# raahii/dcvgan

Hardware: AMD Instinct MI355X
Metric: videos/sec per G+D step, 16x64x64 RGB+depth (higher is better)
Workload: dtype f32

## Files before the change

### dcvgan_amd/csrc/conv_mfma.hip

```cpp
#include "dcv_common.h"

#include <algorithm>
#include <cstdlib>
#include <map>
#include <mutex>
#include <string>
#include <type_traits>
#include <vector>

namespace dcv {

thread_local char g_err[512] = {0};
std::atomic<uint64_t> g_launches{0};
thread_local char g_last_kernel[160] = {0};
#define DCV_NOTE_KERNEL(...) snprintf(g_last_kernel, sizeof(g_last_kernel), __VA_ARGS__)

typedef float f32x16 __attribute__((ext_vector_type(16)));
typedef __bf16 bf16x8 __attribute__((ext_vector_type(8)));

std::atomic<int> g_precision{0};
struct BnView {
    const float* bx; const float* gamma; const float* beta; const float* mean; const float* invstd;
    int64_t bx_sn;
    int32_t bx_sc, bx_sh, cbn, act;
    float slope;
};

__device__ __forceinline__ bf16x8 pack_bf16x8(const float (&t)[8]) {
// ... 1661 lines not shown
                if (accumulate) { v[0] += dst[0]; v[1] += dst[1]; }
                dst[0] = apply_act(v[0], act, slope);
                dst[1] = apply_act(v[1], act, slope);
            }
}

template <int T>
static bool launch_thin_struct(const GatherArgs& a, int OC, int RC, int rc_per_split, dim3 grid, hipStream_t s) {
    switch (OC) {
        case 1: hipLaunchKernelGGL((thin_struct_kernel<T, 1>), grid, dim3(256), 0, s, a, RC, rc_per_split); return true;
        case 2: hipLaunchKernelGGL((thin_struct_kernel<T, 2>), grid, dim3(256), 0, s, a, RC, rc_per_split); return true;
        case 3: hipLaunchKernelGGL((thin_struct_kernel<T, 3>), grid, dim3(256), 0, s, a, RC, rc_per_split); return true;
        case 4: hipLaunchKernelGGL((thin_struct_kernel<T, 4>), grid, dim3(256), 0, s, a, RC, rc_per_split); return true;
    }
    return false;
}

struct PackArgs {
    const KEntry* ktab[4];
    float* wp[4];
    int32_t K16[4];
    int32_t fmt[4];
};
__global__ void pack_weights_kernel(const float* __restrict__ w, const PackArgs pa, int OC, int OCp, int64_t ws_o) {
    const int c = blockIdx.y;
    const int64_t i = (int64_t)blockIdx.x * blockDim.x + threadIdx.x;
    if (i >= (int64_t)pa.K16[c] * OCp) return;
    const int k = (int)(i / OCp), oc = (int)(i % OCp);
    const KEntry e = pa.ktab[c][k];
    float v = 0.f;
    if (oc < OC && !(e.tapsel >> 31)) v = w[(int64_t)oc * ws_o + e.w_off];
    if (pa.fmt[c] == 2) {
        if (X6_PHASE(k >> 4)) v = -v;
        __bf16* o = reinterpret_cast<__bf16*>(pa.wp[c]);
        const __bf16 hi = (__bf16)v;
        const float r = v - (float)hi;
        const __bf16 mid = (__bf16)r;
        const __bf16 lo = (__bf16)(r - (float)mid);
        const int64_t base = (((int64_t)(k >> 4) * 6 + ((k >> 3) & 1)) * OCp + oc) * 8 + (k & 7);
        o[base] = hi; o[base + (int64_t)2 * OCp * 8] = mid; o[base + (int64_t)4 * OCp * 8] = lo;
    } else if (pa.fmt[c]) reinterpret_cast<__bf16*>(pa.wp[c])[((int64_t)(k >> 3) * OCp + oc) * 8 + (k & 7)] = (__bf16)v;
    else pa.wp[c][i] = v;
}

struct WgradArgs {
    const float* dptr;
    const float* gptr;
    float* slab;
    const KEntry* jtab;
    int32_t M, DC, J, DCp, Jp, chunk, pad0, pad1;
    FastDiv div_sp, div_hw, div_w;
    DimTaps td, th, tw;
    int64_t d_sn, g_sn;
    int32_t d_sc4, d_sd, d_sh, d_sw;
    int32_t g_sd, g_sh, g_sw, pad2;
    int32_t g_sc4, g_sd4, log2nd, pad3;
    int32_t hw_off4[16];
    uint32_t hw_sel[16];
};

template <int TD, int TJ, int WD, int WJ, bool REG16>
__global__ __launch_bounds__(256, (TD * TJ >= 4 ? (REG16 ? 3 : 2) : 3)) void wgrad_gemm_kernel(const WgradArgs a) {
    constexpr int BD = 32 * TD * WD;
    constexpr int BJ = 32 * TJ * WJ;
    constexpr int DPT = BD / 8, JPT = BJ / 8;
// ... 1035 lines not shown
            if (lane == 0 && c0 + cc < a.C)
                out[(int64_t)(c0 + cc) * (ND * 16) + (e >> 2) * 16 + ((1 - ph) + 2 * ((e >> 1) & 1)) * 4 + (1 - pw) + 2 * (e & 1)] = v;
        }
}
#undef DCV_HEAD_LANES

struct DevTable {
    KEntry* dev = nullptr;
    int32_t* koff = nullptr;
    uint32_t* ksel = nullptr;
    int rows = 0;
};

static std::mutex g_plan_mu;
static std::map<std::string, DevTable> g_tables;

struct Toggles {
    bool no_lds_dma, no_dstep, no_patch, no_row64, no_widen, no_widen_mfma, no_thinj_wgrad, no_wgrad_dma, no_wgrad_dma64, no_quad, no_thin_wgrad;
    int half_m;
    bool no_ragged, no_wgrad_d16, no_head_kernels, no_stem3d_wgrad, wgrad_x6;
    int stem3d_stages;
#ifdef DCV_DEBUG_TIMING
    bool debug_nostore;
#endif
    Toggles() {
        auto on = [](const char* n) { return getenv(n) != nullptr; };
        no_lds_dma = on("DCV_NO_LDS_DMA"); no_dstep = on("DCV_NO_DSTEP"); no_patch = on("DCV_NO_PATCH"); no_row64 = on("DCV_NO_ROW64");
        no_widen = on("DCV_NO_WIDEN"); no_widen_mfma = on("DCV_NO_WIDEN_MFMA"); no_thinj_wgrad = on("DCV_NO_THINJ_WGRAD"); no_wgrad_dma = on("DCV_NO_WGRAD_DMA"); no_wgrad_dma64 = on("DCV_NO_WGRAD_DMA64"); no_quad = on("DCV_NO_QUAD"); no_thin_wgrad = on("DCV_NO_THIN_WGRAD");
        half_m = getenv("DCV_HALF_M") ? atoi(getenv("DCV_HALF_M")) : -1;
        no_ragged = on("DCV_NO_RAGGED");
        no_wgrad_d16 = on("DCV_NO_WGRAD_D16");
        no_head_kernels = on("DCV_NO_HEAD_KERNELS"); no_stem3d_wgrad = on("DCV_NO_STEM3D_WGRAD"); wgrad_x6 = on("DCV_WGRAD_X6");
        stem3d_stages = getenv("DCV_STEM3D_STAGES") ? atoi(getenv("DCV_STEM3D_STAGES")) : 0;
#ifdef DCV_DEBUG_TIMING
        debug_nostore = on("DCV_DEBUG_NOSTORE");
#endif
    }
};
static const Toggles& toggles() {
    static const Toggles t;
    return t;
}

struct HeadBnRequest {
    int mode;
    const float* bx; dcv_dims5 bxd; float* bdx; dcv_dims5 bdxd;
    const float* gamma; const float* beta; const float* mean; const float* invstd;
    const float* cst; float* partial; size_t partial_bytes;
    int cbn; float slope;
};

struct CallOpts {
    int precision = 0;
    int wgrad_acc = 0;
    const BnView* bnview = nullptr;
    const HeadBnRequest* headbn = nullptr;
};
static int call_opts(const dcv_conv_geom* g, CallOpts* o, const char* tag) {
// ... 622 lines not shown
        GatherArgsPack one;
        for (int i = 0; i < 4; ++i) one.c[i] = a;
        hipLaunchKernelGGL(splitk_reduce_kernel, dim3((unsigned)((tot + 255) / 256), 1), dim3(256), 0, stream, one, KS2);
        break;
    }
    }
    DCV_LAUNCH_CHECK();
    return DCV_OK;
}

static int run_gather(const GatherOp& op, const GatherPlan& P, const CallOpts& o, const dcv_wpack* pack, void* ws, hipStream_t stream) {
    const TileCfg& tc = P.tc;
    const bool own_pack = pack && pack->buf;
    char* const wp_base = static_cast<char*>(own_pack ? pack->buf : ws);
    const bool pk_ready = own_pack && pack->ready;
    if (P.stat_memset) DCV_HIP_CHECK(hipMemsetAsync(op.stat, 0, P.stat_need, stream));
    GatherArgsPack pend;
    PackArgs packs;
    memset(&packs, 0, sizeof(packs));
    int npack = 0, packmax = 0, npend = 0, KSpend = 1;
    dim3 pend_grid(0, 1, 1);
    auto flush_pk = [&]() {
        if (npack == 0) return (int)DCV_OK;
        const int rc = flush_packs(op.w, packs, npack, packmax, op.OC, P.OCp, op.ws_o, stream);
        npack = packmax = 0;
        return rc;
    };
    auto flush_pend = [&]() {
        int rc = flush_pk();
        if (rc == DCV_OK && npend > 0) rc = flush_pending(pend, npend, pend_grid, tc, KSpend, op.OC, o.precision, stream);
        npend = 0;
        return rc;
    };
    for (const ClassPlan& cp : P.cls) {
        DevTable tab;
        int rc = gather_table(op, cp, &tab);
        if (rc != DCV_OK) return rc;
        GatherArgs a = cp.a;
        float* const wp = reinterpret_cast<float*>(wp_base + cp.wp_off);
        a.x = op.x; a.y = op.y; a.wp = wp; a.koff = tab.koff; a.ksel = tab.ksel; a.gate = op.gate;
        a.slab = cp.KS2 > 1 ? reinterpret_cast<float*>(static_cast<char*>(ws) + cp.slab_off) : nullptr;
        a.stat = cp.stat ? op.stat : nullptr;
        if (!pk_ready) {
            packs.ktab[npack] = tab.dev; packs.wp[npack] = wp; packs.K16[npack] = a.KIT * 16; packs.fmt[npack] = cp.fmt;
            packmax = std::max(packmax, a.KIT * 16);
            if (++npack == 4 && (rc = flush_pk()) != DCV_OK) return rc;
// ... 760 lines not shown
    HeadBnRequest hb{1, bn_x, *bn_xd, bn_dx, *bn_dxd, gamma, beta, save_mean, save_invstd, cst, static_cast<float*>(ws2), pbytes, cbn, act == DCV_ACT_LEAKY ? slope : 1.f};
    o.headbn = &hb;
    ConvCall c; ConvPlan P;
    c.which = 1; c.g = g; c.xd = dxd; c.yd = dyd; c.src = dy; c.w = w; c.dst = dx; c.pack = pack;
    if ((rc = plan_conv(c, o, &P)) != DCV_OK) return rc;
    const bool fuse = P.path == ConvPath::Gather && P.gp.cls.size() == 1 && P.gp.cls[0].kind == GK::HeadBn;
    if ((rc = run_conv(c, P, o, ws, ws_bytes, stream)) != DCV_OK || !fuse) return rc;
    const double count = (double)bn_xd->n * bn_xd->d * bn_xd->h * bn_xd->w;
    hipLaunchKernelGGL(head_bn_finalize_kernel, dim3(cbn), dim3(256), 0, static_cast<hipStream_t>(stream), hb.partial, (int)P.gp.cls[0].grid.x, cbn, count, gamma, save_invstd, dgamma, dbeta, cst);
    DCV_LAUNCH_CHECK();
    hb.mode = 2;
    dcv_wpack pk2;
    if (pack && pack->buf) { pk2 = *pack; pk2.ready = 1; c.pack = &pk2; }
    if ((rc = run_conv(c, P, o, ws, ws_bytes, stream)) != DCV_OK) return rc;
    *fused = 1;
    return DCV_OK;
}

size_t dcv_conv_packed_bytes(const dcv_conv_geom* g, const dcv_dims5* x, const dcv_dims5* y, int which) {
    ConvPlan P;
    return (which == 0 || which == 1) && plan_sizes(g, x, y, which, false, &P) == DCV_OK ? P.gp.pack_need : 0;
}

int dcv_conv_forward(const dcv_conv_geom* g, const float* x, const dcv_dims5* xd, const float* w, float* y, const dcv_dims5* yd,
                     int act, float slope, const dcv_wpack* pack, void* ws, size_t ws_bytes, void* stream) {
    ConvCall c;
    c.g = g; c.xd = xd; c.yd = yd; c.src = x; c.w = w; c.dst = y; c.act = act; c.slope = slope; c.pack = pack;
    return conv_call(c, ws, ws_bytes, stream);
}

size_t dcv_conv_stats_bytes(const dcv_conv_geom* g, const dcv_dims5* x, const dcv_dims5* y) {
    ConvPlan P;
    return plan_sizes(g, x, y, 0, true, &P) == DCV_OK && P.op.stats ? P.gp.stat_need : 0;
}

int dcv_conv_forward_stats(const dcv_conv_geom* g, const float* x, const dcv_dims5* xd, const float* w, float* y, const dcv_dims5* yd,
                           float* stat, size_t stat_bytes, int* nparts, int* pitch, const dcv_wpack* pack, void* ws, size_t ws_bytes, void* stream) {
    if (!stat || !nparts || !pitch) return fail(DCV_EINVAL, "conv_forward_stats: null pointer");
    CallOpts o; ConvCall c; ConvPlan P;
    int rc = call_opts(g, &o, "conv");
    if (rc != DCV_OK) return rc;
    c.g = g; c.xd = xd; c.yd = yd; c.src = x; c.w = w; c.dst = y; c.pack = pack;
    c.stats = true; c.stat = stat; c.stat_bytes = stat_bytes;
    if ((rc = plan_conv(c, o, &P)) != DCV_OK) return rc;
    *pitch = P.gp.OCp;
    return run_conv(c, P, o, ws, ws_bytes, stream, nparts);
// ... 84 lines not shown
```

### dcvgan_amd/native.py

```python
from __future__ import annotations

import ctypes as C
import os
import threading
from typing import Optional, Sequence

import torch

_HERE = os.path.dirname(os.path.abspath(__file__))
LIB_PATH = os.environ.get("DCV_LIB_PATH") or os.path.join(_HERE, "libdcvgan_hip.so")

ACT_NONE, ACT_LEAKY, ACT_TANH = 0, 1, 2
DCV_OK, DCV_EINVAL, DCV_EWORKSPACE, DCV_EHIP, DCV_EUNSUPPORTED = 0, -1, -2, -3, -4


class NativeError(RuntimeError):
    pass


class Dims5(C.Structure):
    _fields_ = [("n", C.c_int32), ("c", C.c_int32), ("d", C.c_int32), ("h", C.c_int32), ("w", C.c_int32),
                ("sn", C.c_int64), ("sc", C.c_int64), ("sd", C.c_int64), ("sh", C.c_int64), ("sw", C.c_int64)]


class WPack(C.Structure):
    _fields_ = [("buf", C.c_void_p), ("bytes", C.c_size_t), ("ready", C.c_int32),
                ("precision", C.c_int32)]


class ConvGeom(C.Structure):
    _fields_ = [("kd", C.c_int32), ("kh", C.c_int32), ("kw", C.c_int32),
                ("sd", C.c_int32), ("sh", C.c_int32), ("sw", C.c_int32),
                ("pd", C.c_int32), ("ph", C.c_int32), ("pw", C.c_int32),
                ("transposed", C.c_int32), ("cin", C.c_int32), ("cout", C.c_int32),
                ("mfma", C.c_int32)]

    def key(self):
        return tuple(getattr(self, f) for f, _ in self._fields_)


class AugLimits(C.Structure):
    _fields_ = [("mx", C.c_int32), ("my", C.c_int32), ("size", C.c_int32), ("mask", C.c_int32), ("contrast", C.c_float), ("brightness", C.c_float)]


class AugWarpLimits(C.Structure):
    _fields_ = [("scale_max", C.c_float), ("aniso_max", C.c_float), ("rot_tan_half", C.c_float), ("frac", C.c_float), ("sat", C.c_float), ("mask", C.c_int32)]


_P = C.c_void_p
_D = C.POINTER(Dims5)
_G = C.POINTER(ConvGeom)
_SIGS = {
    "dcv_last_error": (C.c_char_p, []),
    "dcv_version": (C.c_int, []),
    "dcv_abi_struct_sizes": (None, [C.POINTER(C.c_size_t)]),
    "dcv_conv_effective_precision": (C.c_int, [_G]),
    "dcv_launch_count": (C.c_uint64, []),
    "dcv_debug_kernel_info": (C.c_int, [C.c_char_p, C.c_size_t]),
    "dcv_debug_last_kernel": (C.c_char_p, []),
    "dcv_set_precision": (C.c_int, [C.c_int]),
    "dcv_get_precision": (C.c_int, []),
    "dcv_conv_workspace_bytes": (C.c_size_t, [_G, _D, _D, C.c_int]),
    "dcv_conv_packed_bytes": (C.c_size_t, [_G, _D, _D, C.c_int]),
    "dcv_conv_forward": (C.c_int, [_G, _P, _D, _P, _P, _D, C.c_int, C.c_float, _P, _P, C.c_size_t, _P]),
    "dcv_conv_stats_bytes": (C.c_size_t, [_G, _D, _D]),
    "dcv_conv_forward_stats": (C.c_int, [_G, _P, _D, _P, _P, _D, _P, C.c_size_t, C.POINTER(C.c_int), C.POINTER(C.c_int), _P, _P, C.c_size_t, _P]),
    "dcv_conv_backward_data": (C.c_int, [_G, _P, _D, _P, _P, _D, C.c_int, _P, _P, C.c_size_t, _P]),
    "dcv_conv_backward_data_gated": (C.c_int, [_G, _P, _D, _P, _P, _D, C.c_int, _P, _D, C.c_int, C.c_float, _P, _P, C.c_size_t, _P]),
    "dcv_bn_forward_stats_only": (C.c_int, [_P, _D, _P, _P, _P, _P, _P, C.c_float, C.c_float, _P, C.c_int, C.c_int, _P]),
    "dcv_bn_apply": (C.c_int, [_P, _D, _P, _D, _P, _P, _P, _P, _P, C.c_int, C.c_float, _P]),
    "dcv_conv_forward_bn": (C.c_int, [_G, _P, _D, _P, _P, _D, C.c_int, C.c_float, _P, _P, C.c_size_t, C.c_int, _P, _D, _P, _P, _P, _P, C.c_int, C.c_float, _P]),
    "dcv_conv_backward_weight_bn": (C.c_int, [_G, _P, _D, _P, _D, _P, C.c_int, _P, C.c_size_t, C.c_int, _P, _D, _P, _P, _P, _P, C.c_int, C.c_float, _P]),
    "dcv_conv_backward_data_bn_workspace_bytes": (C.c_size_t, [_D, C.c_int]),
    "dcv_conv_backward_data_bn": (C.c_int, [_G, _P, _D, _P, _P, _D, _P, _P, C.c_size_t, C.c_int, _P, _D, _P, _P, _P, _P, C.c_int, C.c_float, _P, _D, _P, _P,
                                            _P, C.c_size_t, C.POINTER(C.c_int), _P]),
    "dcv_conv_backward_weight": (C.c_int, [_G, _P, _D, _P, _D, _P, _P, C.c_size_t, _P]),
    "dcv_conv_backward_weight_acc": (C.c_int, [_G, _P, _D, _P, _D, _P, C.c_int, _P, C.c_size_t, _P]),
    "dcv_bn_workspace_bytes": (C.c_size_t, [C.c_int]),
    "dcv_bn_act_forward": (C.c_int, [_P, _D, _P, _D, _P, _P, _P, _P, _P, _P, _P, _P, C.c_int, C.c_float, C.c_float, C.c_int, C.c_float, _P, C.c_size_t, _P]),
    "dcv_bn_act_forward_stats": (C.c_int, [_P, _D, _P, _D, _P, _P, _P, _P, _P, _P, _P, _P, C.c_float, C.c_float, C.c_int, C.c_float, _P, C.c_int, C.c_int, _P, C.c_size_t, _P]),
    "dcv_bn_act_backward": (C.c_int, [_P, _D, _P, _D, _P, _D, _P, _P, _P, _P, _P, C.c_int, C.c_int, C.c_float, _P, _P, _P, C.c_size_t, _P]),
    "dcv_act_forward": (C.c_int, [_P, _D, _P, _D, C.c_int, C.c_float, _P]),
    "dcv_act_backward": (C.c_int, [_P, _D, _P, _D, _P, _D, C.c_int, C.c_float, _P]),
    "dcv_axpby": (C.c_int, [_P, _D, C.c_float, _P, _D, C.c_float, _P, _D, _P]),
    "dcv_noise_add": (C.c_int, [_P, _D, _P, _D, C.c_float, C.c_uint64, C.c_uint64, _P]),
    "dcv_normal_fill": (C.c_int, [_P, C.c_int64, C.c_uint64, C.c_uint64, _P]),
# ... 242 lines not shown
```

### dcvgan_amd/ops.py

```python
from __future__ import annotations

import collections
import ctypes as C
import os
from typing import Optional, Tuple

import torch
from torch.autograd import Function

from . import native as N
from .native import ACT_LEAKY, ACT_NONE, ACT_TANH, ConvGeom, check, dims5, lib, ptr, stream_ptr

__all__ = ["invalidate_packed_weights", "conv", "bn_act", "sync_bn_act", "act", "noise_add", "cat_channels", "temporal_diff", "gan_loss", "gru_sequence",
           "normal", "dropout2d_mask", "conv_geom", "ACT_NONE", "ACT_LEAKY", "ACT_TANH"]


def _dense(t: torch.Tensor) -> torch.Tensor:
    if any(s == 0 and n > 1 for s, n in zip(t.stride(), t.shape)):
        return t.contiguous()
    return t


_POISON = bool(int(os.environ.get("DCV_DEBUG_POISON", "0")))
_USE_PACK_CACHE = os.environ.get("DCV_NO_PACK_CACHE") is None
_WGRAD_SIDE = os.environ.get("DCV_NO_WGRAD_SIDE") is None
_HEAD_BN_DEFER = os.environ.get("DCV_NO_HEAD_BN_DEFER") is None
_SKIP_ACCUMULATE = True
_GATED_DGRAD = True
_OWN_ACCUMULATION = True
_HEAD_BN_FUSION = True


def _empty(shape, device) -> torch.Tensor:
    if _POISON:
        return torch.full(tuple(shape), float("nan"), dtype=torch.float32, device=device)
    return torch.empty(tuple(shape), dtype=torch.float32, device=device)
# ... 38 lines not shown
class _Opaque:
    __slots__ = ("v",)

    def __init__(self, v):
        self.v = v


def _dest(out, shape, device):
    if out is None:
        return _empty(shape, device)
    t = out.t
    if tuple(t.shape) != tuple(shape):
        raise N.NativeError(f"out= has shape {tuple(t.shape)}, expected {tuple(shape)}")
    N._require(t, "out= destination")
    return t.detach()


class _PackCache:
    __slots__ = ("entries",)

    def __init__(self):
        self.entries = {}

    def get(self, w, which, g, xd_t, yd_t, xd, yd):
        prec = lib().dcv_conv_effective_precision(C.byref(g))
        key = (which, g.key(), prec, tuple(xd_t.shape), tuple(xd_t.stride()), tuple(yd_t.shape), tuple(yd_t.stride()))
        e = self.entries.get(key)
        stamp = (w._version, w.data_ptr(), prec)
        if _POISON:
            wd = w.detach().double()
            stamp = stamp + (float(wd.sum()), float(wd.abs().sum()))
        if e is None:
            nbytes = lib().dcv_conv_packed_bytes(C.byref(g), C.byref(xd), C.byref(yd), which)
            if nbytes == 0:
                return None
            e = self.entries[key] = [None, torch.empty(nbytes, dtype=torch.uint8, device=w.device), None, None]
        ready = e[0] == stamp
        if w.is_cuda:
            cur = torch.cuda.current_stream(w.device)
            if e[2] is not None and e[3] != cur.cuda_stream:
                cur.wait_event(e[2])
        e[0] = None
        pk = N.WPack(e[1].data_ptr(), e[1].numel(), int(ready), prec)
        pk._entry, pk._stamp, pk._packs = e, stamp, not ready
        return pk

    @staticmethod
    def commit(pk):
        if pk is not None:
            e = pk._entry
            e[0] = pk._stamp
            if pk._packs and e[1].is_cuda:
                cur = torch.cuda.current_stream(e[1].device)
                if e[2] is None:
                    e[2] = torch.cuda.Event()
                e[2].record(cur)
                e[3] = cur.cuda_stream


def _pack_of(w):
    if not _USE_PACK_CACHE:
        return None
    pc = getattr(w, "_dcv_pack", None)
    if pc is None:
        pc = w._dcv_pack = _PackCache()
    return pc


def invalidate_packed_weights(obj) -> None:
    ts = obj.parameters() if isinstance(obj, torch.nn.Module) else [obj]
    for t in ts:
        if getattr(t, "_dcv_pack", None) is not None:
            t._dcv_pack = None


def _task_id() -> int:
    return torch._C._current_graph_task_id()


def _engine_accumulates(p) -> bool:
    tid = _task_id()
    if tid < 0:
        return True
    c = getattr(p, "_dcv_engine", None)
    if c is not None and c[0] == tid:
        return c[1]
    with torch.enable_grad():
        node = p.view_as(p).grad_fn.next_functions[0][0]
    try:
        ok = bool(torch._C._will_engine_execute_node(node))
    except RuntimeError:
        ok = False
    p._dcv_engine = (tid, ok)
    return ok


# ... 809 lines not shown
```

### dcvgan_amd/optim.py

```python
from __future__ import annotations

import ctypes as C
from typing import Iterable, List, Optional

import torch

from .native import NativeError, PointerTable, _require, c_array, check, lib, ptr, stream_ptr


class GradGuard:

    FIELDS = ("loss_scale", "growth_tracker", "grad_norm", "clip_coef", "factor", "skipped", "skipped_total", "nonfinite")

    def __init__(self, max_norm: Optional[float] = None, skip_nonfinite: bool = True, loss_scale: float = 1.0, dynamic: bool = False,
                 growth_factor: float = 2.0, backoff_factor: float = 0.5, growth_interval: int = 2000):
        import math
        if max_norm is not None and not (float(max_norm) > 0.0 and math.isfinite(float(max_norm))):
            raise ValueError(f"GradGuard: max_norm must be a positive finite number or None, got {max_norm!r}")
        if not (float(loss_scale) > 0.0 and math.isfinite(float(loss_scale))):
            raise ValueError(f"GradGuard: loss_scale must be positive and finite, got {loss_scale!r}")
        if not float(growth_factor) > 1.0:
            raise ValueError(f"GradGuard: growth_factor must be > 1, got {growth_factor!r}")
        if not 0.0 < float(backoff_factor) < 1.0:
            raise ValueError(f"GradGuard: backoff_factor must be in (0, 1), got {backoff_factor!r}")
# ... 59 lines not shown
            w.inner.grad_scale = 1.0 / w.world
        scales = {o.grad_scale for o in self.optimizers}
        if len(scales) != 1:
            raise NativeError(f"GradGuard: the registered optimisers disagree on grad_scale ({sorted(scales)})")
        gs, ns, keep = [], [], []
        for o in self.optimizers:
            for p in o.params:
                g = p.grad
                if g is None or g.numel() == 0:
                    continue
                _require(g, "GradGuard gradient")
                g = g.contiguous()
                gs.append(g.data_ptr()); ns.append(g.numel()); keep.append(g)
        tab = self._tables = PointerTable.cached(self._tables, (tuple(gs), tuple(ns)),
                                                 lambda: dict(n=len(gs), g=c_array(gs), numel=c_array(ns, C.c_int64)))
        L = lib()
        need = L.dcv_grad_guard_workspace_bytes(sum(ns), tab.n)
        if self._ws is None or self._ws.numel() < need:
            self._ws = torch.empty(need, dtype=torch.uint8, device=state.device)
        check(L.dcv_grad_guard_measure(tab.n, tab.g, tab.numel, scales.pop(), self.max_norm if self.max_norm is not None else 0.0, int(self.skip_nonfinite), int(self.dynamic),
                                       self.growth_factor, self.backoff_factor, self.growth_interval, ptr(state), ptr(self._ws), self._ws.numel(), stream_ptr()),
              "dcv_grad_guard_measure")
        self.measurements += 1


class Adam:
    def __init__(self, params: Iterable[torch.nn.Parameter], lr: float = 1e-3, betas=(0.9, 0.999), eps: float = 1e-8, weight_decay: float = 0.0,
                 guard: Optional[GradGuard] = None):
        self.params: List[torch.nn.Parameter] = [p for p in params]
        if not self.params:
            raise ValueError("optimizer got an empty parameter list")
        self.lr, self.betas, self.eps, self.weight_decay = float(lr), (float(betas[0]), float(betas[1])), float(eps), float(weight_decay)
        self.state = {}
        self.grad_scale = 1.0
        self.guard = guard
        if guard is not None:
            guard._register(self)

    def zero_grad(self, set_to_none: bool = True):
        for p in self.params:
            if set_to_none:
                p.grad = None
            elif p.grad is not None:
                p.grad.zero_()

    def state_dict(self):
# ... 51 lines not shown
        groups, touched, fresh = {}, [], None
        for p in self.params:
            g = p.grad
            if g is None:
                continue
            _require(p.data, "Adam parameter")
            if not p.data.is_contiguous():
                raise NativeError("Adam: parameters must be contiguous")
            g = g.contiguous()
            s = self.state.get(p)
            if s is None:
                if fresh is None:
                    fresh = torch.zeros(16, dtype=torch.int32, device=p.device)
                s = self.state[p] = {"step": fresh[0], "step_block": fresh, "exp_avg": torch.zeros_like(p.data), "exp_avg_sq": torch.zeros_like(p.data)}
            touched.append(p)
            grp = groups.setdefault(s["step_block"].data_ptr(), ([], [], [], [], [], []))
            grp[0].append(p.data.data_ptr()); grp[1].append(g.data_ptr()); grp[2].append(s["exp_avg"].data_ptr()); grp[3].append(s["exp_avg_sq"].data_ptr())
            grp[4].append(p.numel()); grp[5].append(g)
        for block, (ps, gs, ms, vs, ns, _) in groups.items():
            check(L.dcv_adam_step_multi_guarded(len(ps), c_array(ps), c_array(gs), c_array(ms), c_array(vs), c_array(ns, C.c_int64), self.lr, self.betas[0], self.betas[1],
                                                self.eps, self.weight_decay, C.c_void_p(block), ptr(guard.state), st), "dcv_adam_step_multi_guarded")
        if touched:
            torch.autograd.graph.increment_version(touched)

    @torch.no_grad()
    def step(self):
        if self.guard is not None:
            return self._step_guarded()
        L = lib()
        st = stream_ptr()
        ps, gs, ms, vs, ns, keep = [], [], [], [], [], []
        touched = []
        step = None
        for p in self.params:
            g = p.grad
            if g is None:
                continue
            _require(p.data, "Adam parameter")
            if not p.data.is_contiguous():
                raise NativeError("Adam: parameters must be contiguous")
            g = g.contiguous()
            s = self.state.get(p)
            if s is None:
                s = self.state[p] = {"step": 0, "exp_avg": torch.zeros_like(p.data), "exp_avg_sq": torch.zeros_like(p.data)}
            s["step"] += 1
            touched.append(p)
            if step is None:
                step = s["step"]
            if s["step"] != step:
                check(L.dcv_adam_step(ptr(p.data), ptr(g), ptr(s["exp_avg"]), ptr(s["exp_avg_sq"]), p.numel(), self.lr, self.betas[0], self.betas[1],
                                      self.eps, self.weight_decay, s["step"], self.grad_scale, st), "dcv_adam_step")
                continue
            ps.append(p.data.data_ptr()); gs.append(g.data_ptr()); ms.append(s["exp_avg"].data_ptr()); vs.append(s["exp_avg_sq"].data_ptr())
            ns.append(p.numel()); keep.append(g)
        if ps:
            check(L.dcv_adam_step_multi(len(ps), c_array(ps), c_array(gs), c_array(ms), c_array(vs), c_array(ns, C.c_int64), self.lr, self.betas[0], self.betas[1],
                                        self.eps, self.weight_decay, step, self.grad_scale, st), "dcv_adam_step_multi")
        if touched:
            torch.autograd.graph.increment_version(touched)


class ModelEma:

    def __init__(self, models, names=("ggen", "cgen"), decay: float = 0.999, warmup: bool = True, guard: Optional[GradGuard] = None):
        if not 0.0 <= float(decay) < 1.0:
            raise ValueError(f"ModelEma: decay must be in [0, 1), got {decay!r}")
        self.names = tuple(names)
        if not self.names:
            raise ValueError("ModelEma: no model names")
        self.decay, self.warmup, self.guard = float(decay), bool(warmup), guard
        from .rng import PhiloxRng
        self.live = {n: models[n] for n in self.names}
        self.rng = PhiloxRng()
        self.twins = {n: self._twin(m, self.rng) for n, m in self.live.items()}
        self._pairs = {}
        for n, m in self.live.items():
            tp, tb = dict(self.twins[n].named_parameters()), dict(self.twins[n].named_buffers())
            self._pairs[n] = [(tp[k], p) for k, p in m.named_parameters()] + [(tb[k], b) for k, b in m.named_buffers()]
        self._n_params = {n: sum(1 for _ in m.parameters()) for n, m in self.live.items()}
        self._tables = {}
        dev = next(self.live[self.names[0]].parameters()).device
        self._blocks = {n: torch.zeros(16, dtype=torch.int32).to(dev) for n in self.names}
# ... 504 lines not shown
                _require(t.data, f"SpectralNorm tensor of convolution {i}")
                if not t.is_contiguous():
                    raise NativeError("SpectralNorm: tensors must be contiguous")
            w, w_sn, u, v, sg = row
            if w_sn.shape != w.shape or u.numel() != w.shape[0] or v.numel() != w[0].numel() or sg.numel() != 1:
                raise NativeError(f"SpectralNorm: the buffers of convolution {i} do not fit its weight {tuple(w.shape)}")
        n = len(ts)
        w, w_sn, u, v, sigma = (c_array(col) for col in zip(*ts))
        rows, cols = c_array([row[0].shape[0] for row in ts], C.c_int32), c_array([row[0][0].numel() for row in ts], C.c_int32)
        need = lib().dcv_spectral_workspace_bytes(n, rows, cols)
        if need == 0:
            raise NativeError("dcv_spectral_workspace_bytes: " + lib().dcv_last_error().decode(errors="replace"))
        if self._ws is None or self._ws.numel() < need:
            self._ws = torch.empty(need, dtype=torch.uint8, device=ts[0][0].device)
        return dict(n=n, w=w, w_sn=w_sn, u=u, v=v, sigma=sigma, rows=rows, cols=cols, touched=[row[1] for row in ts])

    @torch.no_grad()
    def update(self, n_iter: int = 1, _guarded: bool = True):
        t = self._table()
        state = ptr(self.guard._need_state()) if (self.guard is not None and _guarded) else None
        check(lib().dcv_spectral_update_multi(t.n, t.w, t.w_sn, t.u, t.v, t.sigma, t.rows, t.cols, int(n_iter), self.eps, state, ptr(self._ws), self._ws.numel(),
                                              stream_ptr()), "dcv_spectral_update_multi")
        torch.autograd.graph.increment_version(t.touched)
        for c in self.convs:
            c.__dict__["_dcv_spectral"].version = c.weight._version

    def refresh(self):
        self.update(n_iter=0, _guarded=False)

    @torch.no_grad()
    def project(self):
        for w in list(self._dp) + (list(self.guard._dp) if self.guard is not None else []):
            w.reduce_gradients()
        t = self._table()
        idx, gs = [], []
        for i, c in enumerate(self.convs):
            g = c.weight.grad
            if g is None:
                continue
            _require(g, "SpectralNorm gradient")
            if not g.is_contiguous() or g.shape != c.weight.shape:
                raise NativeError("SpectralNorm: gradients must be contiguous and of the weight's shape")
            idx.append(i); gs.append(g.data_ptr())
        if not idx:
            return
        pick = lambda arr, ty=C.c_void_p: c_array([arr[i] for i in idx], ty)
# ... 27 lines not shown
```

### dcvgan_amd/trainer.py

```python
from __future__ import annotations

import collections
import os
from typing import Dict, Optional

import torch

from . import discriminator as D
from . import generator as G
from . import loss as Lm
from . import ops, optim, util
from .configs import StepConfig

MODEL_NAMES = ("ggen", "cgen", "idis", "vdis", "gdis")


def build_models(cfg: StepConfig, device=None, sync_bn: bool = False) -> Dict[str, torch.nn.Module]:
    w = cfg.width
    ggen = G.GeometricVideoGenerator(cfg.dim_z_content, cfg.dim_z_motion, cfg.channel, cfg.geometric_info, w["ggen"], cfg.video_length)
    cgen = G.ColorVideoGenerator(ggen.channel, cfg.dim_z_color, cfg.geometric_info, w["cgen"], cfg.video_length)
    idis = D.ImageDiscriminator(ggen.channel, cgen.channel, cfg.use_noise["idis"], cfg.noise_sigma["idis"], w["idis"])
    vdis = D.VideoDiscriminator(ggen.channel, cgen.channel, cfg.use_noise["vdis"], cfg.noise_sigma["vdis"], w["vdis"])
    gdis = D.GradientDiscriminator(ggen.channel, cgen.channel, cfg.use_noise["gdis"], cfg.noise_sigma["gdis"], w["gdis"])
    models = dict(ggen=ggen, cgen=cgen, idis=idis, vdis=vdis, gdis=gdis)
# ... 202 lines not shown
            xg_fake, xc_fake = self._colour(cgen, xg_fake, t_rand)
        self._mark("D: generators forward (beside D on the real batch)")
        y_fake = self._fakes_through(dis, idis, xg_fake, xc_fake, t_rand)
        self._adopt(y_real)
        if self.augment is not None:
            for y in y_real:
                self.augment.observe(y)
        self._mark("D: discriminators forward on the fakes")
        if self.lecam is not None:
            loss_idis, loss_vdis, loss_gdis = self.lecam.compute_dis_losses(self.loss, y_real, y_fake)
        else:
            loss_idis = self.loss.compute_dis_loss(y_real[0], y_fake[0])
            loss_vdis = self.loss.compute_dis_loss(y_real[1], y_fake[1])
            loss_gdis = self.loss.compute_dis_loss(y_real[2], y_fake[2])
        loss_dis = ops.sum_scalars(loss_idis, loss_vdis, loss_gdis) if loss_idis.is_cuda else loss_idis + loss_vdis + loss_gdis
        d_steps = self.iteration % c.num_gen_update == 0
        if d_steps:
            loss_dis.backward(guard_dis.root(loss_dis) if guard_dis is not None else self._root(loss_dis))
            self._mark("D: backward (D lanes, then the generators' dead backward)")
            if self.spectral is not None:
                self.spectral.project()
            if guard_dis is not None:
                guard_dis.measure()
            o["idis"].step(); o["vdis"].step(); o["gdis"].step()
            if self.spectral is not None:
                self.spectral.update()
            self._mark("D: Adam")
        else:
            loss_dis.detach_()
        if self.sync_losses:
            out = {"loss_idis": loss_idis.cpu().item(), "loss_vdis": loss_vdis.cpu().item(), "loss_gdis": loss_gdis.cpu().item()}
        else:
            out = {"loss_idis": loss_idis.detach(), "loss_vdis": loss_vdis.detach(), "loss_gdis": loss_gdis.detach()}
        if self.lecam is not None:
            reg = self.lecam.reg.cpu().tolist() if self.sync_losses else self.lecam.reg
            out["lecam_idis"], out["lecam_vdis"], out["lecam_gdis"] = reg[0], reg[1], reg[2]
        if guard_dis is not None:
            self._guard_report(out, guard_dis, "dis")
        if self.augment is not None:
            self.augment.end_of_iteration(self.iteration)
        if self.monitor is not None:
            seen = {f"{n}_real": y.detach() for n, y in zip(("idis", "vdis", "gdis"), y_real)}
            seen.update({f"{n}_fake_d": y.detach() for n, y in zip(("idis", "vdis", "gdis"), y_fake)})
        del y_real, y_fake, xg_fake, xc_fake, loss_dis
        ggen.train(); cgen.train()
        ggen.zero_grad(); cgen.zero_grad()
        xg_fake = ggen.sample_videos(c.batchsize)
        xg_fake, xc_fake = self._colour(cgen, xg_fake, t_rand)
        self._mark("G: generators forward")
        y_fake = self._fakes_through(dis, idis, xg_fake, xc_fake, t_rand)
        loss_gen = self.loss.compute_gen_loss(*y_fake)
        self._mark("G: discriminators forward on the fakes")
        g_steps = self.iteration % c.num_dis_update == 0
        if g_steps:
            loss_gen.backward(guard_gen.root(loss_gen) if guard_gen is not None else self._root(loss_gen))
            self._mark("G: backward (D lanes, then the generators)")
            if guard_gen is not None:
                guard_gen.measure()
            o["ggen"].step(); o["cgen"].step(); o["ggen"].step()
            if self.ema is not None:
                self.ema.update()
            self._mark("G: Adam")
        else:
            loss_gen.detach_()
        out["loss_gen"] = loss_gen.cpu().item() if self.sync_losses else loss_gen.detach()
        if guard_gen is not None:
            self._guard_report(out, guard_gen, "gen")
        if self.monitor is not None:
            seen.update({f"{n}_fake_g": y.detach() for n, y in zip(("idis", "vdis", "gdis"), y_fake)})
            gated = ([] if d_steps else ["grad_norm_dis", "skipped_dis"]) + ([] if g_steps else ["grad_norm_gen", "skipped_gen"])
            self.monitor.observe({k: v for k, v in out.items() if k not in gated}, seen)
            if self.iteration % self.monitor.interval == 0:
                self.monitor.roll(self.iteration)
            del seen
        if xc_real.is_cuda:
            e = torch.cuda.Event()
            e.record(torch.cuda.current_stream())
            self._inflight.append(e)
        return out
```

### include/dcvgan_hip.h

```cpp
#ifndef DCVGAN_HIP_H
#define DCVGAN_HIP_H

#include <stddef.h>
#include <stdint.h>

#ifdef __cplusplus
extern "C" {
#endif

#define DCV_OK 0
#define DCV_EINVAL (-1)
#define DCV_EWORKSPACE (-2)
#define DCV_EHIP (-3)
#define DCV_EUNSUPPORTED (-4)

#define DCV_ACT_NONE 0
#define DCV_ACT_LEAKY 1
#define DCV_ACT_TANH 2

typedef struct dcv_dims5 {
    int32_t n, c, d, h, w;
    int64_t sn, sc, sd, sh, sw;
} dcv_dims5;

// ... 4 lines not shown
    int32_t transposed;
    int32_t cin, cout;
    int32_t mfma;
} dcv_conv_geom;

const char* dcv_last_error(void);
int dcv_version(void);
void dcv_abi_struct_sizes(size_t out[3]);
uint64_t dcv_launch_count(void);
int dcv_set_precision(int mode);
int dcv_get_precision(void);
int dcv_conv_effective_precision(const dcv_conv_geom* g);
const char* dcv_debug_last_kernel(void);
int dcv_debug_kernel_info(char* buf, size_t n);

size_t dcv_conv_workspace_bytes(const dcv_conv_geom* g, const dcv_dims5* x, const dcv_dims5* y, int which );
typedef struct dcv_wpack {
    float* buf;
    size_t bytes;
    int32_t ready;
    int32_t precision;
} dcv_wpack;
size_t dcv_conv_packed_bytes(const dcv_conv_geom* g, const dcv_dims5* x, const dcv_dims5* y, int which );
int dcv_conv_forward(const dcv_conv_geom* g, const float* x, const dcv_dims5* xd, const float* w,
                     float* y, const dcv_dims5* yd, int act, float slope, const dcv_wpack* pack,
                     void* ws, size_t ws_bytes, void* stream);
size_t dcv_conv_stats_bytes(const dcv_conv_geom* g, const dcv_dims5* x, const dcv_dims5* y);
int dcv_conv_forward_stats(const dcv_conv_geom* g, const float* x, const dcv_dims5* xd, const float* w, float* y, const dcv_dims5* yd,
                           float* stat, size_t stat_bytes, int* nparts, int* pitch, const dcv_wpack* pack, void* ws, size_t ws_bytes, void* stream);
int dcv_conv_backward_data(const dcv_conv_geom* g, const float* dy, const dcv_dims5* dyd, const float* w,
                           float* dx, const dcv_dims5* dxd, int accumulate, const dcv_wpack* pack,
                           void* ws, size_t ws_bytes, void* stream);
int dcv_conv_backward_data_gated(const dcv_conv_geom* g, const float* dy, const dcv_dims5* dyd, const float* w,
                                 float* dx, const dcv_dims5* dxd, int accumulate,
                                 const float* x, const dcv_dims5* xd, int act, float slope, const dcv_wpack* pack,
                                 void* ws, size_t ws_bytes, void* stream);
int dcv_bn_forward_stats_only(const float* x, const dcv_dims5* xd, float* running_mean, float* running_var, int64_t* num_batches_tracked, float* save_mean, float* save_invstd,
                              float momentum, float eps, const float* stat, int nparts, int pitch, void* stream);
int dcv_bn_apply(const float* x, const dcv_dims5* xd, float* y, const dcv_dims5* yd, const float* gamma, const float* beta, const float* save_mean, const float* save_invstd,
                 const float* mask, int act, float slope, void* stream);
int dcv_conv_forward_bn(const dcv_conv_geom* g, const float* x, const dcv_dims5* xd, const float* w, float* y, const dcv_dims5* yd, int act, float slope,
                        const dcv_wpack* pack, void* ws, size_t ws_bytes, int cbn, const float* bn_x, const dcv_dims5* bn_xd, const float* gamma, const float* beta,
                        const float* save_mean, const float* save_invstd, int bn_act, float bn_slope, void* stream);
int dcv_conv_backward_weight_bn(const dcv_conv_geom* g, const float* x, const dcv_dims5* xd, const float* dy, const dcv_dims5* dyd, float* dw, int accumulate,
                                void* ws, size_t ws_bytes, int cbn, const float* bn_x, const dcv_dims5* bn_xd, const float* gamma, const float* beta,
                                const float* save_mean, const float* save_invstd, int bn_act, float bn_slope, void* stream);
// ... 306 lines not shown
```

Measured before the change: 661.2.

## Batch weight repacking into one multi-job kernel launched after optimizer steps

Adds dcv_conv_pack_many, which repacks every cached conv weight touched by the Adam and spectral steps in a single launch. A cached device job table is binary-searched per block. The optimizers call refresh_packed and the trainer groups them with refresh_group, so the per-conv pack launches that used to run lazily inside the next forward pass are skipped. This trades many small launches and their host overhead for one grouped launch, plus extra bookkeeping (stamps and refresh counts) in the pack cache.

```diff
diff --git a/dcvgan_amd/csrc/conv_mfma.hip b/dcvgan_amd/csrc/conv_mfma.hip
--- a/dcvgan_amd/csrc/conv_mfma.hip
+++ b/dcvgan_amd/csrc/conv_mfma.hip
@@ -4,6 +4,7 @@
 #include <cstdlib>
 #include <map>
 #include <mutex>
+#include <set>
 #include <string>
 #include <type_traits>
 #include <vector>
@@ -1711,25 +1712,49 @@
     int32_t K16[4];
     int32_t fmt[4];
 };
-__global__ void pack_weights_kernel(const float* __restrict__ w, const PackArgs pa, int OC, int OCp, int64_t ws_o) {
-    const int c = blockIdx.y;
-    const int64_t i = (int64_t)blockIdx.x * blockDim.x + threadIdx.x;
-    if (i >= (int64_t)pa.K16[c] * OCp) return;
+__device__ __forceinline__ void pack_weights_element(const float* __restrict__ w, const KEntry* __restrict__ ktab, float* __restrict__ wp, int K16, int fmt,
+                                                     int OC, int OCp, int64_t ws_o, int64_t i) {
+    if (i >= (int64_t)K16 * OCp) return;
     const int k = (int)(i / OCp), oc = (int)(i % OCp);
-    const KEntry e = pa.ktab[c][k];
+    const KEntry e = ktab[k];
     float v = 0.f;
     if (oc < OC && !(e.tapsel >> 31)) v = w[(int64_t)oc * ws_o + e.w_off];
-    if (pa.fmt[c] == 2) {
+    if (fmt == 2) {
         if (X6_PHASE(k >> 4)) v = -v;
-        __bf16* o = reinterpret_cast<__bf16*>(pa.wp[c]);
+        __bf16* o = reinterpret_cast<__bf16*>(wp);
         const __bf16 hi = (__bf16)v;
         const float r = v - (float)hi;
         const __bf16 mid = (__bf16)r;
         const __bf16 lo = (__bf16)(r - (float)mid);
         const int64_t base = (((int64_t)(k >> 4) * 6 + ((k >> 3) & 1)) * OCp + oc) * 8 + (k & 7);
         o[base] = hi; o[base + (int64_t)2 * OCp * 8] = mid; o[base + (int64_t)4 * OCp * 8] = lo;
-    } else if (pa.fmt[c]) reinterpret_cast<__bf16*>(pa.wp[c])[((int64_t)(k >> 3) * OCp + oc) * 8 + (k & 7)] = (__bf16)v;
-    else pa.wp[c][i] = v;
+    } else if (fmt) reinterpret_cast<__bf16*>(wp)[((int64_t)(k >> 3) * OCp + oc) * 8 + (k & 7)] = (__bf16)v;
+    else wp[i] = v;
+}
+__global__ void pack_weights_kernel(const float* __restrict__ w, const PackArgs pa, int OC, int OCp, int64_t ws_o) {
+    const int c = blockIdx.y;
+    pack_weights_element(w, pa.ktab[c], pa.wp[c], pa.K16[c], pa.fmt[c], OC, OCp, ws_o, (int64_t)blockIdx.x * blockDim.x + threadIdx.x);
+}
+
+struct PackJob {
+    const float* w;
+    PackArgs pa;
+    int64_t ws_o;
+    int32_t n, OC, OCp;
+    uint32_t bx, block0;
+    int32_t pad;
+};
+__global__ __launch_bounds__(256) void pack_weights_many_kernel(const PackJob* __restrict__ jobs, int njobs) {
+    int lo = 0, hi = njobs - 1;
+    while (lo < hi) {
+        const int mid = (lo + hi + 1) >> 1;
+        if (jobs[mid].block0 <= blockIdx.x) lo = mid; else hi = mid - 1;
+    }
+    const PackJob& j = jobs[lo];
+    const uint32_t lb = blockIdx.x - j.block0;
+    const int c = (int)(lb / j.bx);
+    if (c >= j.n) return;
+    pack_weights_element(j.w, j.pa.ktab[c], j.pa.wp[c], j.pa.K16[c], j.pa.fmt[c], j.OC, j.OCp, j.ws_o, (int64_t)(lb % j.bx) * 256 + threadIdx.x);
 }
 
 struct WgradArgs {
@@ -2811,6 +2836,7 @@
     int stem3d_stages;
 #ifdef DCV_DEBUG_TIMING
     bool debug_nostore;
+    bool debug_skip_repack;
 #endif
     Toggles() {
         auto on = [](const char* n) { return getenv(n) != nullptr; };
@@ -2823,6 +2849,7 @@
         stem3d_stages = getenv("DCV_STEM3D_STAGES") ? atoi(getenv("DCV_STEM3D_STAGES")) : 0;
 #ifdef DCV_DEBUG_TIMING
         debug_nostore = on("DCV_DEBUG_NOSTORE");
+        debug_skip_repack = getenv("DCV_SKIP_GROUP") && !strcmp(getenv("DCV_SKIP_GROUP"), "repack");
 #endif
     }
 };
@@ -3491,6 +3518,14 @@
     dim3 pend_grid(0, 1, 1);
     auto flush_pk = [&]() {
         if (npack == 0) return (int)DCV_OK;
+#ifdef DCV_DEBUG_TIMING
+        if (toggles().debug_skip_repack && own_pack) {
+            static std::mutex mu;
+            static std::set<const void*> filled;
+            std::lock_guard<std::mutex> lk(mu);
+            if (!filled.insert(packs.wp[0]).second) { npack = packmax = 0; return (int)DCV_OK; }
+        }
+#endif
         const int rc = flush_packs(op.w, packs, npack, packmax, op.OC, P.OCp, op.ws_o, stream);
         npack = packmax = 0;
         return rc;
@@ -4297,6 +4332,93 @@
     return (which == 0 || which == 1) && plan_sizes(g, x, y, which, false, &P) == DCV_OK ? P.gp.pack_need : 0;
 }
 
+struct PackTable { PackJob* dev = nullptr; int njobs = 0; unsigned blocks = 0; };
+static std::mutex g_pack_mu;
+static std::map<std::string, PackTable> g_pack_tables;
+
+static int build_pack_jobs(int n, const dcv_pack_item* items, std::vector<PackJob>* jobs, unsigned* blocks) {
+    uint64_t total = 0;
+    for (int i = 0; i < n; ++i) {
+        const dcv_pack_item& it = items[i];
+        CallOpts o; ConvCall c; ConvPlan P;
+        c.which = it.which; c.g = &it.g; c.xd = &it.x; c.yd = &it.y; c.w = it.w; c.pack = &it.pack;
+        int rc = call_opts(&it.g, &o, "conv_pack_many");
+        if (rc == DCV_OK) rc = plan_conv(c, o, &P, true);
+        if (rc != DCV_OK) return rc;
+        if (P.gp.pack_need > it.pack.bytes)
+            return fail(DCV_EWORKSPACE, "conv_pack_many: packed-weight buffer of item %d too small (%zu needed, %zu given)", i, P.gp.pack_need, it.pack.bytes);
+        PackJob job;
+        memset(&job, 0, sizeof(job));
+        int kmax = 0;
+        auto close = [&]() {
+            if (job.n == 0) return;
+            job.w = it.w; job.OC = P.op.OC; job.OCp = P.gp.OCp; job.ws_o = P.op.ws_o;
+            job.bx = (unsigned)(((int64_t)kmax * P.gp.OCp + 255) / 256);
+            job.block0 = (uint32_t)total;
+            total += (uint64_t)job.bx * job.n;
+            jobs->push_back(job);
+            memset(&job, 0, sizeof(job));
+            kmax = 0;
+        };
+        for (const ClassPlan& cp : P.gp.cls) {
+            DevTable tab;
+            if ((rc = gather_table(P.op, cp, &tab)) != DCV_OK) return rc;
+            job.pa.ktab[job.n] = tab.dev; job.pa.wp[job.n] = reinterpret_cast<float*>(reinterpret_cast<char*>(it.pack.buf) + cp.wp_off);
+            job.pa.K16[job.n] = cp.a.KIT * 16; job.pa.fmt[job.n] = cp.fmt;
+            kmax = std::max(kmax, cp.a.KIT * 16);
+            if (++job.n == 4) close();
+        }
+        close();
+        if (total >= (1ull << 31)) return fail(DCV_EUNSUPPORTED, "conv_pack_many: too many elements for one launch");
+    }
+    *blocks = (unsigned)total;
+    return DCV_OK;
+}
+
+int dcv_conv_pack_many(int n, const dcv_pack_item* items, size_t item_bytes, void* stream) {
+    if (n < 0 || (n > 0 && !items) || item_bytes != sizeof(dcv_pack_item))
+        return fail(DCV_EINVAL, "conv_pack_many: bad arguments (n %d, item size %zu, this library's dcv_pack_item has %zu bytes)", n, item_bytes, sizeof(dcv_pack_item));
+    if (n == 0) return DCV_OK;
+    for (int i = 0; i < n; ++i) {
+        const dcv_pack_item& it = items[i];
+        if (!it.w || !it.pack.buf || (it.which != 0 && it.which != 1)) return fail(DCV_EINVAL, "conv_pack_many: item %d: null pointer or bad pass", i);
+        CallOpts o;
+        const int rc = call_opts(&it.g, &o, "conv_pack_many");
+        if (rc != DCV_OK) return rc;
+        if (it.pack.precision != o.precision + 1)
+            return fail(DCV_EINVAL, "conv_pack_many: item %d: dcv_wpack.precision is %d but its convolution runs at precision %d", i, it.pack.precision, o.precision + 1);
+    }
+    std::string key = device_prefix();
+    key.append(reinterpret_cast<const char*>(items), (size_t)n * sizeof(dcv_pack_item));
+    PackTable t;
+    {
+        std::lock_guard<std::mutex> lk(g_pack_mu);
+        auto f = g_pack_tables.find(key);
+        if (f != g_pack_tables.end()) t = f->second;
+        else {
+            std::vector<PackJob> jobs;
+            const int rc = build_pack_jobs(n, items, &jobs, &t.blocks);
+            if (rc != DCV_OK) return rc;
+            if (jobs.empty() || t.blocks == 0) return DCV_OK;
+            if (g_pack_tables.size() >= 64) {
+                for (auto& kv : g_pack_tables) (void)hipFree(kv.second.dev);
+                g_pack_tables.clear();
+            }
+            t.njobs = (int)jobs.size();
+            DCV_HIP_CHECK(hipMalloc((void**)&t.dev, jobs.size() * sizeof(PackJob)));
+            const hipError_t e = hipMemcpy(t.dev, jobs.data(), jobs.size() * sizeof(PackJob), hipMemcpyHostToDevice);
+            if (e != hipSuccess) {
+                (void)hipFree(t.dev);
+                return fail(DCV_EHIP, "conv_pack_many: uploading the job table failed: %s", hipGetErrorString(e));
+            }
+            g_pack_tables[key] = t;
+        }
+    }
+    hipLaunchKernelGGL(pack_weights_many_kernel, dim3(t.blocks), dim3(256), 0, static_cast<hipStream_t>(stream), t.dev, t.njobs);
+    DCV_LAUNCH_CHECK();
+    return DCV_OK;
+}
+
 int dcv_conv_forward(const dcv_conv_geom* g, const float* x, const dcv_dims5* xd, const float* w, float* y, const dcv_dims5* yd,
                      int act, float slope, const dcv_wpack* pack, void* ws, size_t ws_bytes, void* stream) {
     ConvCall c;
diff --git a/dcvgan_amd/native.py b/dcvgan_amd/native.py
--- a/dcvgan_amd/native.py
+++ b/dcvgan_amd/native.py
@@ -37,6 +37,10 @@
 
     def key(self):
         return tuple(getattr(self, f) for f, _ in self._fields_)
+
+
+class PackItem(C.Structure):
+    _fields_ = [("w", C.c_void_p), ("g", ConvGeom), ("x", Dims5), ("y", Dims5), ("which", C.c_int32), ("pack", WPack)]
 
 
 class AugLimits(C.Structure):
@@ -62,6 +66,7 @@
     "dcv_get_precision": (C.c_int, []),
     "dcv_conv_workspace_bytes": (C.c_size_t, [_G, _D, _D, C.c_int]),
     "dcv_conv_packed_bytes": (C.c_size_t, [_G, _D, _D, C.c_int]),
+    "dcv_conv_pack_many": (C.c_int, [C.c_int, C.POINTER(PackItem), C.c_size_t, _P]),
     "dcv_conv_forward": (C.c_int, [_G, _P, _D, _P, _P, _D, C.c_int, C.c_float, _P, _P, C.c_size_t, _P]),
     "dcv_conv_stats_bytes": (C.c_size_t, [_G, _D, _D]),
     "dcv_conv_forward_stats": (C.c_int, [_G, _P, _D, _P, _P, _D, _P, C.c_size_t, C.POINTER(C.c_int), C.POINTER(C.c_int), _P, _P, C.c_size_t, _P]),
diff --git a/dcvgan_amd/ops.py b/dcvgan_amd/ops.py
--- a/dcvgan_amd/ops.py
+++ b/dcvgan_amd/ops.py
@@ -3,6 +3,7 @@
 import collections
 import ctypes as C
 import os
+import threading
 from typing import Optional, Tuple
 
 import torch
@@ -11,7 +12,7 @@
 from . import native as N
 from .native import ACT_LEAKY, ACT_NONE, ACT_TANH, ConvGeom, check, dims5, lib, ptr, stream_ptr
 
-__all__ = ["invalidate_packed_weights", "conv", "bn_act", "sync_bn_act", "act", "noise_add", "cat_channels", "temporal_diff", "gan_loss", "gru_sequence",
+__all__ = ["invalidate_packed_weights", "refresh_packed", "refresh_group", "conv", "bn_act", "sync_bn_act", "act", "noise_add", "cat_channels", "temporal_diff", "gan_loss", "gru_sequence",
            "normal", "dropout2d_mask", "conv_geom", "ACT_NONE", "ACT_LEAKY", "ACT_TANH"]
 
 
@@ -96,19 +97,24 @@
     def __init__(self):
         self.entries = {}
 
+    @staticmethod
+    def stamp(w, prec):
+        s = (w._version, w.data_ptr(), prec)
+        if _POISON:
+            wd = w.detach().double()
+            s = s + (float(wd.sum()), float(wd.abs().sum()))
+        return s
+
     def get(self, w, which, g, xd_t, yd_t, xd, yd):
         prec = lib().dcv_conv_effective_precision(C.byref(g))
         key = (which, g.key(), prec, tuple(xd_t.shape), tuple(xd_t.stride()), tuple(yd_t.shape), tuple(yd_t.stride()))
         e = self.entries.get(key)
-        stamp = (w._version, w.data_ptr(), prec)
-        if _POISON:
-            wd = w.detach().double()
-            stamp = stamp + (float(wd.sum()), float(wd.abs().sum()))
+        stamp = self.stamp(w, prec)
         if e is None:
             nbytes = lib().dcv_conv_packed_bytes(C.byref(g), C.byref(xd), C.byref(yd), which)
             if nbytes == 0:
                 return None
-            e = self.entries[key] = [None, torch.empty(nbytes, dtype=torch.uint8, device=w.device), None, None]
+            e = self.entries[key] = [None, torch.empty(nbytes, dtype=torch.uint8, device=w.device), None, None, 0, (which, ConvGeom(*g.key()), xd, yd, prec), False]
         ready = e[0] == stamp
         if w.is_cuda:
             cur = torch.cuda.current_stream(w.device)
@@ -124,10 +130,11 @@
         if pk is not None:
             e = pk._entry
             e[0] = pk._stamp
+            e[4] = 0
             if pk._packs and e[1].is_cuda:
                 cur = torch.cuda.current_stream(e[1].device)
-                if e[2] is None:
-                    e[2] = torch.cuda.Event()
+                if e[2] is None or e[6]:
+                    e[2], e[6] = torch.cuda.Event(), False
                 e[2].record(cur)
                 e[3] = cur.cuda_stream
 
@@ -146,6 +153,67 @@
     for t in ts:
         if getattr(t, "_dcv_pack", None) is not None:
             t._dcv_pack = None
+
+
+_refresh_tls = threading.local()
+_refresh_items = {}
+
+
+class refresh_group:
+    def __enter__(self):
+        self.outer = getattr(_refresh_tls, "pending", None)
+        if self.outer is None:
+            _refresh_tls.pending = []
+        return self
+
+    def __exit__(self, exc_type, exc, tb):
+        if self.outer is None:
+            pending, _refresh_tls.pending = _refresh_tls.pending, None
+            if exc_type is None:
+                refresh_packed(pending)
+        return False
+
+
+def refresh_packed(tensors) -> int:
+    tensors = list(tensors)
+    pending = getattr(_refresh_tls, "pending", None)
+    if pending is not None:
+        pending.extend(tensors)
+        return N.DCV_OK
+    found, key, seen = [], [], set()
+    for w in tensors:
+        pc = getattr(w, "_dcv_pack", None)
+        if pc is None or id(w) in seen or not _USE_PACK_CACHE or not w.is_cuda or w.device.index != torch.cuda.current_device():
+            continue
+        seen.add(id(w))
+        for k, e in pc.entries.items():
+            which, g, xd, yd, prec = e[5]
+            if e[4] < 2 and lib().dcv_conv_effective_precision(C.byref(g)) == prec:
+                found.append((w, e))
+                key.append((w.data_ptr(), e[1].data_ptr(), e[1].numel(), k))
+    if not found:
+        return N.DCV_OK
+    key = tuple(key)
+    tab = _refresh_items.get(key)
+    if tab is None:
+        if len(_refresh_items) >= 32:
+            _refresh_items.clear()
+        items = (N.PackItem * len(found))()
+        for it, (w, e) in zip(items, found):
+            which, g, xd, yd, prec = e[5]
+            it.w, it.g, it.x, it.y, it.which, it.pack = w.data_ptr(), g, xd, yd, which, N.WPack(e[1].data_ptr(), e[1].numel(), 0, prec)
+        tab = _refresh_items[key] = items
+    rc = lib().dcv_conv_pack_many(len(found), tab, C.sizeof(N.PackItem), stream_ptr())
+    if rc != N.DCV_OK:
+        if rc == N.DCV_EHIP:
+            check(rc, "dcv_conv_pack_many")
+        return rc
+    cur = torch.cuda.current_stream(found[0][0].device)
+    ev = torch.cuda.Event()
+    ev.record(cur)
+    for w, e in found:
+        e[0], e[2], e[3], e[4], e[6] = _PackCache.stamp(w, e[5][4]), ev, cur.cuda_stream, e[4] + 1, True
+    return rc
 
 
 def _task_id() -> int:
diff --git a/dcvgan_amd/optim.py b/dcvgan_amd/optim.py
--- a/dcvgan_amd/optim.py
+++ b/dcvgan_amd/optim.py
@@ -105,6 +105,11 @@
                                        self.growth_factor, self.backoff_factor, self.growth_interval, ptr(state), ptr(self._ws), self._ws.numel(), stream_ptr()),
               "dcv_grad_guard_measure")
         self.measurements += 1
+
+
+def _refresh_packed(tensors):
+    from . import ops
+    ops.refresh_packed(tensors)
 
 
 class Adam:
@@ -202,6 +207,7 @@
                                                 self.eps, self.weight_decay, C.c_void_p(block), ptr(guard.state), st), "dcv_adam_step_multi_guarded")
         if touched:
             torch.autograd.graph.increment_version(touched)
+            _refresh_packed(touched)
 
     @torch.no_grad()
     def step(self):
@@ -238,6 +244,7 @@
                                         self.eps, self.weight_decay, step, self.grad_scale, st), "dcv_adam_step_multi")
         if touched:
             torch.autograd.graph.increment_version(touched)
+            _refresh_packed(touched)
 
 
 class ModelEma:
@@ -788,6 +795,7 @@
         check(lib().dcv_spectral_update_multi(t.n, t.w, t.w_sn, t.u, t.v, t.sigma, t.rows, t.cols, int(n_iter), self.eps, state, ptr(self._ws), self._ws.numel(),
                                               stream_ptr()), "dcv_spectral_update_multi")
         torch.autograd.graph.increment_version(t.touched)
+        _refresh_packed(t.touched)
         for c in self.convs:
             c.__dict__["_dcv_spectral"].version = c.weight._version
 
diff --git a/dcvgan_amd/trainer.py b/dcvgan_amd/trainer.py
--- a/dcvgan_amd/trainer.py
+++ b/dcvgan_amd/trainer.py
@@ -248,9 +248,10 @@
                 self.spectral.project()
             if guard_dis is not None:
                 guard_dis.measure()
-            o["idis"].step(); o["vdis"].step(); o["gdis"].step()
-            if self.spectral is not None:
-                self.spectral.update()
+            with ops.refresh_group():
+                o["idis"].step(); o["vdis"].step(); o["gdis"].step()
+                if self.spectral is not None:
+                    self.spectral.update()
             self._mark("D: Adam")
         else:
             loss_dis.detach_()
@@ -283,7 +284,8 @@
             self._mark("G: backward (D lanes, then the generators)")
             if guard_gen is not None:
                 guard_gen.measure()
-            o["ggen"].step(); o["cgen"].step(); o["ggen"].step()
+            with ops.refresh_group():
+                o["ggen"].step(); o["cgen"].step(); o["ggen"].step()
             if self.ema is not None:
                 self.ema.update()
             self._mark("G: Adam")
diff --git a/include/dcvgan_hip.h b/include/dcvgan_hip.h
--- a/include/dcvgan_hip.h
+++ b/include/dcvgan_hip.h
@@ -50,6 +50,14 @@
     int32_t precision;
 } dcv_wpack;
 size_t dcv_conv_packed_bytes(const dcv_conv_geom* g, const dcv_dims5* x, const dcv_dims5* y, int which );
+typedef struct dcv_pack_item {
+    const float* w;
+    dcv_conv_geom g;
+    dcv_dims5 x, y;
+    int32_t which;
+    dcv_wpack pack;
+} dcv_pack_item;
+int dcv_conv_pack_many(int n, const dcv_pack_item* items, size_t item_bytes, void* stream);
 int dcv_conv_forward(const dcv_conv_geom* g, const float* x, const dcv_dims5* xd, const float* w,
                      float* y, const dcv_dims5* yd, int act, float slope, const dcv_wpack* pack,
                      void* ws, size_t ws_bytes, void* stream);
```

Result: no change. 664.3, median of 6 (+0.5%).
